# askerlee/AdaFace-dev

Hardware: AMD Instinct MI355X
Metric: denoise-steps/sec SD-1.5 U-Net 512px bs=4/GPU (higher is better)
Workload: dtype f16; 1 GPU; adaface_txt2img_ddim: SD-1.5 U-Net eps-prediction + CFG + DDIM update, 512x512 (latent 64x64), bs=4/GPU, U-Net batch 8 (cond+uncond), 77 tokens, DDIM-50 timesteps, random-init weights; parallelism=replicas x1, hipgraph=True, finite=True

## Files before the change

### adaface-dev_amd/_lib.py

```python
import ctypes as C
import os
import subprocess

_HERE = os.path.dirname(os.path.abspath(__file__))
CSRC = os.path.join(_HERE, "csrc")
LIB_PATH = os.environ.get("AF_LIB") or os.path.join(CSRC, "libadaface_hip.so")

AF_OK, AF_E_BADARG, AF_E_UNSUPPORTED, AF_E_HIP = 0, -1, -2, -3
AF_ACT_NONE, AF_ACT_SILU, AF_ACT_GEGLU, AF_ACT_QUICKGELU = 0, 1, 2, 3
AF_OUT_NORMAL, AF_OUT_SPLIT_T, AF_OUT_F32 = 0, 1, 2
AF_SPLITK_COUNTER_BYTES = 4096 * 4
AF_FAM_GEMM, AF_FAM_ATTN, AF_FAM_GNORM, AF_FAM_LNORM, AF_FAM_ELEM, AF_FAM_XATTN = 0, 1, 2, 3, 4, 5

EXPORTS = (
    "af_last_error", "af_version", "af_device_count", "af_prof_enable", "af_prof_reset", "af_prof_read",
    "af_gemm", "af_groupnorm_ws_floats", "af_groupnorm", "af_layernorm", "af_attention", "af_attention_scores",
    "af_timestep_embedding", "af_nchw_f32_to_nhwc_f16", "af_nhwc_f16_to_nchw_f32", "af_cfg_ddim_step", "af_q_sample",
    "af_silu_f16", "af_attention_lse", "af_groupnorm_stats", "af_attention_bwd_scratch_bytes", "af_attention_bwd",
    "af_groupnorm_bwd", "af_layernorm_bwd", "af_geglu_fwd", "af_geglu_bwd", "af_sumpool2x2", "af_add_f16",
    "af_transpose_tokens", "af_cadamw_step", "af_attention_ex", "af_colsum", "af_quickgelu_fwd", "af_quickgelu_bwd",
    "af_scale_f32", "af_affine_prelu", "af_maxpool2x2", "af_global_avgpool", "af_se_residual_prelu", "af_axpy_f16", "af_dora_combine", "af_mul_f16", "af_im2col3x3", "af_colsum_tall", "af_softmax_rows", "af_attention_strided", "af_clamp_f32", "af_mask_pairs", "af_prefetch", "af_prefetch_ex",
    "af_xattn_scores", "af_xattn_softmax_pv", "af_xattn_softmax_pv_bwd", "af_xattn_rowmix", "af_xattn_colmix_ws_bytes", "af_xattn_colmix",
    "af_layernorm_param_grads", "af_transpose_tokens_pair", "af_ff_fused", "af_ff_chain", "af_xattn_fused",
    "af_softmax_rows_bwd", "af_affine_prelu_bwd", "af_maxpool2x2_bwd", "af_se_gate_grad", "af_se_residual_prelu_bwd",
    "af_groupnorm_apply", "af_gemm_gn_stats_ok", "af_gemm_halo_variant", "af_gn_proj_fused",
    "af_xattn_chain",
    "af_image_u8_to_nhwc_f16", "af_vae_latents_q_sample", "af_cfg_dpmpp_step", "af_cfg_lcm_step",
    "af_cfg_ddim_inpaint_step", "af_cfg_dpmpp_inpaint_step", "af_cfg_lcm_inpaint_step", "af_vae_latents_z_q_sample",
    "af_vae_attention", "af_latent_resize_q_sample", "af_affine_prelu_ch", "af_face_align_crop",
    "af_stem_im2col7x7", "af_relu_maxpool3x3s2", "af_subsample2x", "af_upsample2x_add", "af_retina_decode", "af_retina_nms",
)


class GemmDesc(C.Structure):
    _fields_ = [
        ("a1", C.c_void_p), ("a2", C.c_void_p), ("wt", C.c_void_p), ("bias", C.c_void_p),
        ("rowbias", C.c_void_p), ("residual", C.c_void_p), ("out", C.c_void_p), ("out2", C.c_void_p),
        ("M", C.c_int32), ("N", C.c_int32), ("K", C.c_int32), ("kpad", C.c_int32), ("taps", C.c_int32),
        ("c1", C.c_int32), ("c2", C.c_int32), ("lda1", C.c_int32), ("lda2", C.c_int32),
        ("B", C.c_int32), ("H", C.c_int32), ("W", C.c_int32), ("Ho", C.c_int32), ("Wo", C.c_int32),
        ("stride", C.c_int32), ("upsample", C.c_int32), ("rows_per_batch", C.c_int32), ("ld_rowbias", C.c_int32),
        ("act", C.c_int32), ("out_mode", C.c_int32), ("ld_out", C.c_int32), ("split_col", C.c_int32),
        ("ld_out2", C.c_int32), ("tile", C.c_int32), ("splits", C.c_int32),
        ("workspace", C.c_void_p), ("workspace_bytes", C.c_int64), ("zeros", C.c_void_p),
        ("tap_shift", C.c_int32), ("splitk_fused", C.c_int32),
        ("ln_colsum", C.c_void_p), ("ln_eps", C.c_float),
        ("a3", C.c_void_p), ("a4", C.c_void_p), ("c3", C.c_int32), ("c4", C.c_int32), ("lda3", C.c_int32), ("lda4", C.c_int32),
        ("gn_partials", C.c_void_p), ("gn_cpg", C.c_int32),
# ... 46 lines not shown
        return _lib
    import torch
    if not os.path.exists(LIB_PATH):
        raise RuntimeError(
            f"{LIB_PATH} not found: the HIP extension is required (no CPU fallback). "
            "Run `python -c 'import __graft_entry__ as g; g.build()'` or `make -C adaface-dev_amd/csrc`."
        )
    L = C.CDLL(LIB_PATH)
    vp, i32, i64, f32 = C.c_void_p, C.c_int, C.c_int64, C.c_float
    L.af_last_error.restype = C.c_char_p
    L.af_last_error.argtypes = []
    L.af_version.argtypes = []
    L.af_device_count.argtypes = []
    L.af_prof_enable.argtypes = [i32]
    L.af_prof_reset.argtypes = []
    L.af_prof_read.argtypes = [i32, C.POINTER(C.c_int), C.POINTER(C.c_double)]
    L.af_gemm.argtypes = [C.POINTER(GemmDesc), vp]
    L.af_groupnorm_ws_floats.argtypes = [i32]
    L.af_groupnorm.argtypes = [vp, vp, i32, i32, vp, vp, vp, i32, i32, i32, f32, i32, vp, vp]
    L.af_groupnorm_apply.argtypes = [vp, i32, vp, vp, vp, vp, i32, i32, i32, f32, i32, vp, i32, vp]
    L.af_gemm_gn_stats_ok.argtypes = [i32, i32, i32, i32, i32, i32, i32, i32]
    L.af_gemm_halo_variant.argtypes = [C.POINTER(GemmDesc)]
    L.af_gn_proj_fused.argtypes = [vp, vp, i32, vp, vp, f32, vp, vp, i32, vp, i32, i32, i32, i32, vp, vp]
    L.af_layernorm.argtypes = [vp, vp, vp, vp, i32, i32, f32, vp]
    L.af_attention.argtypes = [vp, vp, vp, vp, vp, i32, i32, i32, i32, i32, i32, i32, i32, i32, i32, f32, vp]
    L.af_attention_scores.argtypes = [vp, vp, vp, vp, i32, i32, i32, i32, i32, f32, vp]
    L.af_timestep_embedding.argtypes = [vp, vp, i32, i32, f32, vp]
    L.af_nchw_f32_to_nhwc_f16.argtypes = [vp, vp, i32, i32, i32, i32, vp]
    L.af_nhwc_f16_to_nchw_f32.argtypes = [vp, vp, i32, i32, i32, i32, vp]
    L.af_cfg_ddim_step.argtypes = [vp, vp, vp, vp, i64, i32, f32, f32, f32, vp]
    L.af_cfg_dpmpp_step.argtypes = [vp, vp, vp, vp, vp, vp, i64, i32, f32, f32, f32, f32, f32, f32, vp]
    L.af_cfg_lcm_step.argtypes = [vp, vp, vp, vp, vp, i64, i32, f32, f32, f32, f32, f32, f32, f32, vp]
    L.af_q_sample.argtypes = [vp, vp, vp, vp, vp, i32, i64, vp]
    L.af_image_u8_to_nhwc_f16.argtypes = [vp, vp, i32, i32, i32, vp]
    L.af_vae_latents_q_sample.argtypes = [vp, vp, vp, vp, vp, f32, f32, f32, vp, i32, i32, i32, i32, vp]
    L.af_vae_latents_z_q_sample.argtypes = [vp, vp, vp, vp, vp, f32, f32, f32, vp, vp, i32, i32, i32, i32, vp]
    L.af_latent_resize_q_sample.argtypes = [vp, vp, vp, i32, i32, i32, i32, i32, i32, f32, f32, vp]
    blend = [vp, vp, vp, i32, i32, i64, f32, f32]
    L.af_cfg_ddim_inpaint_step.argtypes = L.af_cfg_ddim_step.argtypes[:-1] + blend + [vp]
    L.af_cfg_dpmpp_inpaint_step.argtypes = L.af_cfg_dpmpp_step.argtypes[:-1] + blend + [vp]
    L.af_cfg_lcm_inpaint_step.argtypes = L.af_cfg_lcm_step.argtypes[:-1] + blend + [vp]
    L.af_silu_f16.argtypes = [vp, vp, i64, vp]
    L.af_attention_lse.argtypes = [vp, vp, vp, vp, vp, i32, vp, i32, i32, i32, i32, i32, i32, i32, i32, i32, i32, f32, vp]
    L.af_attention_ex.argtypes = [vp, vp, vp, vp, vp, i32, vp, i32, i32, i32, i32, i32, i32, i32, i32, i32, i32, i32, f32, vp]
    L.af_attention_strided.argtypes = [vp, vp, vp, vp, vp, i32, vp, i32, i32, i32, i32, i32, i32, i32, i32, i32, i32, i32, i64, f32, vp]
    L.af_groupnorm_stats.argtypes = [vp, vp, i32, i32, vp, vp, vp, vp, i32, i32, i32, f32, i32, vp, vp]
# ... 68 lines not shown
```

### adaface-dev_amd/csrc/af_xattn_fused.hip

```cpp
#include <stdlib.h>

#include "af_common.h"

namespace {

__device__ __forceinline__ void glds16(const half_t* src, char* lds_dst) {
  __builtin_amdgcn_global_load_lds((const __attribute__((address_space(1))) void*)src,
                                   (__attribute__((address_space(3))) void*)lds_dst, 16, 0, 0);
}

constexpr int XA_C = 320, XA_H = 8, XA_D = 40, XA_BM = 128;
constexpr int XA_WQ = 5 * 48 * 128, XA_WO = XA_C * 128, XA_KB = 80 * 128, XA_VB = 2 * 48 * 128;
constexpr int XA_LDS = XA_WQ + 2 * (XA_WO + XA_KB + XA_VB) + 2 * XA_C * 4;

struct XaDev {
  const half_t* x;
  const half_t* wq;
  const float* bq;
  const float* cs;
  const half_t* k;
  const half_t* vt;
  const half_t* wo;
  const float* bo;
  const half_t* residual;
// ... 1039 lines not shown
#pragma unroll
      for (int tm = 0; tm < 4; ++tm) xf[tm] = *reinterpret_cast<const half8_t*>(Xs + frag_off(wm * 64 + tm * 16, kk));
#pragma unroll
      for (int tn = 0; tn < 5; ++tn)
#pragma unroll
        for (int tm = 0; tm < 4; ++tm) acc[tn][tm] = __builtin_amdgcn_mfma_f32_16x16x32_f16(wf[tn], xf[tm], acc[tn][tm], 0, 0, 0);
    }
  }
#pragma unroll
  for (int tm = 0; tm < 4; ++tm) {
    const int m = m0 + wm * 64 + tm * 16 + fr;
    if (m >= p.M) continue;
#pragma unroll
    for (int tn = 0; tn < 5; ++tn) {
      const int c = wn * 80 + tn * 16 + 4 * fq;
      floatx4 v = acc[tn][tm];
      if (p.bias) {
        const floatx4 b = *reinterpret_cast<const floatx4*>(p.bias + c);
#pragma unroll
        for (int e = 0; e < 4; ++e) v[e] += b[e];
      }
      const half4_t o = {(half_t)v[0], (half_t)v[1], (half_t)v[2], (half_t)v[3]};
      *reinterpret_cast<half4_t*>(p.out + (size_t)m * XA_C + c) = o;
    }
  }
}

}

extern "C" int af_xattn_fused(const void* x, const void* wq, const void* bq, const void* ln_colsum, float ln_eps, int kpad_q, const void* k, int ldk,
                              const void* vt, int64_t vt_batch_stride, int ldv, const void* wo, const void* bo, int kpad_o, const void* residual,
                              void* out, int B, int N, int L, int C, int heads, float scale, const void* zeros, void* stream) {
  AF_REQUIRE(x && wq && k && vt && wo && out && zeros, "af_xattn_fused: null pointer");
  AF_SUPPORTED((C == XA_C || C == X6_C) && heads == XA_H, "af_xattn_fused: built for C = 320 / 640, 8 heads (the 64 x 64 and 32 x 32 levels of SD-1.5)");
  AF_REQUIRE(B > 0 && N > 0 && N % (C == XA_C ? XA_BM : X6_BM) == 0, "af_xattn_fused: tokens per image must be a positive multiple of 128 (C = 320) / 64 (C = 640)");
  AF_SUPPORTED(L > 0 && L <= 80, "af_xattn_fused: at most 80 keys");
  AF_REQUIRE(kpad_q >= C && kpad_q % 64 == 0 && kpad_o >= C && kpad_o % 64 == 0, "af_xattn_fused: weight row strides must be 64-multiples covering C");
  AF_REQUIRE(ldk >= C && ldk % 8 == 0 && ldv >= L && ldv % 8 == 0 && vt_batch_stride % 8 == 0, "af_xattn_fused: K / V^T strides must keep 16-byte alignment");
  XaDev p{};
  p.x = (const half_t*)x;
  p.wq = (const half_t*)wq;
  p.bq = (const float*)bq;
  p.cs = (const float*)ln_colsum;
  p.ln_on = ln_colsum != nullptr;
  p.k = (const half_t*)k;
  p.vt = (const half_t*)vt;
// ... 92 lines not shown
  AF_REQUIRE(B > 0 && HW > 0 && HW % XA_BM == 0 && nblk == HW / XA_BM && nblk <= 128, "af_gn_proj_fused: HW must be a multiple of 128 (at most 128 blocks) and nblk = HW / 128");
  AF_REQUIRE(kpad >= C && kpad % 64 == 0, "af_gn_proj_fused: the weight row stride must be a 64-multiple covering C");
  AF_REQUIRE((((uintptr_t)x | (uintptr_t)out | (uintptr_t)gamma | (uintptr_t)beta | (uintptr_t)w) & 15) == 0, "af_gn_proj_fused: x / out / gamma / beta / w must be 16-byte aligned");
  GpDev p;
  p.x = (const half_t*)x;
  p.partials = (const float*)partials;
  p.gamma = (const float*)gamma;
  p.beta = (const float*)beta;
  p.w = (const half_t*)w;
  p.bias = (const float*)bias;
  p.out = (half_t*)out;
  p.zeros = (const half_t*)zeros;
  p.M = B * HW;
  p.HW = HW;
  p.nblk = nblk;
  p.kpad = kpad;
  p.eps = eps;
  static bool attr_set = false;
  if (!af_allow_dyn_lds(reinterpret_cast<const void*>(&af_gn_proj320_kernel), XT_LDS, attr_set, "af_gn_proj_fused")) return af_check_launch("af_gn_proj_fused");
  AfLaunchScope scope(AF_FAM_GEMM, stream);
  hipLaunchKernelGGL(af_gn_proj320_kernel, dim3(p.M / XA_BM), dim3(512), XT_LDS, (hipStream_t)stream, p);
  return af_check_launch("af_gn_proj_fused");
}
```

### adaface-dev_amd/ldm/modules/attention.py

```python
import math
import os as _os

import torch
import torch.nn as nn
import torch.nn.functional as F

from ... import ops
from ...ops import AF_ACT_GEGLU, F16
from .diffusionmodules.util import (Conv2d, GroupNorm32, LayerNorm, Linear, _PackCache, checkpoint, from_nhwc_f16,
                                    to_nhwc_f16, zero_module)


FOLD_LAYERNORM = _os.environ.get("AF_FOLD_LAYERNORM", "1") != "0"
FUSE_GN_PROJ = _os.environ.get("AF_FUSE_GN_PROJ", "1") != "0"
CHAIN_XATTN = _os.environ.get("AF_CHAIN_XATTN", "1") != "0"
XATTN_FUSE_MIN_TOKENS = int(_os.environ.get("AF_XATTN_FUSE_MIN_TOKENS", "8192"))
CHAIN_PROJ_OUT = _os.environ.get("AF_CHAIN_PROJ_OUT", "1") != "0"
FUSE_XATTN640 = _os.environ.get("AF_FUSE_XATTN640", "0") != "0"
XATTN640_FUSE_MIN_TOKENS = 4096
FUSE_XATTN = _os.environ.get("AF_FUSE_XATTN", "1") != "0"
FUSE_FF = _os.environ.get("AF_FUSE_FF", "1") != "0"


def exists(val):
    return val is not None


def default(val, d):
    if exists(val):
        return val
    return d() if callable(d) else d


def Normalize(in_channels):
    return GroupNorm32(num_groups=32, num_channels=in_channels, eps=1e-6, affine=True)


# ... 113 lines not shown
        ws = (self.to_k.weight, self.to_v.weight)
        return self._kv_cache.get(ws, lambda: ops.pack_matrix(torch.cat([w.detach() for w in ws], 0), None, ws[0].device))

    def _packed_qkv_ln(self, ln):
        ws = (self.to_q.weight, self.to_k.weight, self.to_v.weight)
        if not hasattr(self, "_qkv_cache_ln"):
            self._qkv_cache_ln = _PackCache()
        return self._qkv_cache_ln.get(ws + (ln.weight, ln.bias), lambda: ops.pack_matrix_ln(
            torch.cat([w.detach() for w in ws], 0), None, ln.weight, ln.bias, ln.eps, ws[0].device))

    def _packed_q_ln(self, ln):
        if not hasattr(self, "_q_cache_ln"):
            self._q_cache_ln = _PackCache()
        return self._q_cache_ln.get((self.to_q.weight, ln.weight, ln.bias), lambda: ops.pack_matrix_ln(
            self.to_q.weight, None, ln.weight, ln.bias, ln.eps, self.to_q.weight.device))

    def xattn_fusable(self, C, B, N, L, ln, chain=False) -> bool:
        if not (FUSE_XATTN and ln is not None and self.heads == 8 and not self.save_cross_attn_vars and L <= 80 and self.inner_dim == C):
            return False
        if C == 320:
            return N % 128 == 0 and B * N >= XATTN_FUSE_MIN_TOKENS
        return bool(FUSE_XATTN640 and not chain and C == 640 and N % 64 == 0 and B * N >= XATTN640_FUSE_MIN_TOKENS)

    def hip(self, x2d, B, N, context=None, keybias=None, residual=None, ln=None, defer_out=False, pre=None):
        Ci, h, d = self.inner_dim, self.heads, self.dim_head
        if context is None:
            if self.to_k.in_features != self.to_q.in_features:
                raise RuntimeError("CrossAttention: context is required (context_dim != query_dim)")
            L = N
            qk, vt = ops.gemm(x2d, self._packed_qkv() if ln is None else self._packed_qkv_ln(ln), rows_per_batch=N, split_col=2 * Ci)
            q, k, ldq, ldk = qk, qk[:, Ci:], 2 * Ci, 2 * Ci
        else:
            L = context.shape[1]
            ldk = Ci
            if self._kv_pre is not None:
                k, vt, ldk = self._kv_pre
            else:
                k, vt = ops.gemm(context.reshape(B * L, context.shape[-1]), self._packed_kv(), rows_per_batch=L, split_col=Ci)
            if pre is not None:
                ao, pw_o1, x0 = pre
                return ops.xattn_chain(ao, pw_o1, x0, self._packed_q_ln(ln), k, vt, self.to_out[0].packed(), B=B, N=N, L=L, heads=h, scale=self.scale, ldk=ldk)
            if keybias is None and self.xattn_fusable(x2d.shape[1], B, N, L, ln):
                return ops.xattn_fused(x2d, self._packed_q_ln(ln), k, vt, self.to_out[0].packed(), B=B, N=N, L=L, heads=h, scale=self.scale,
                                       ldk=ldk, residual=residual)
            q = self.to_q.hip(x2d) if ln is None else ops.gemm(x2d, self._packed_q_ln(ln))
            ldq = Ci
        o = ops.attention(q, k, vt, B=B, Nq=N, L=L, heads=h, d=d, ldq=ldq, ldk=ldk, keybias=keybias, scale=self.scale)
        if self.save_cross_attn_vars:
            out_plain = self.to_out[0].hip(o)
            qc = q if context is not None else qk[:, :Ci].contiguous()
            kc = k.contiguous() if context is not None else qk[:, Ci:].contiguous()
            score, prob = ops.attention_scores(qc, kc, B=B, Nq=N, L=L, heads=h, d=d, scale=self.scale)
            rs = math.sqrt(self.scale)
# ... 60 lines not shown
        return self.to_q.hip_dgrad(dq), dctx

    def forward(self, x, context=None, mask=None):
        B, N, _ = x.shape
        x2d = x.reshape(B * N, -1).to(F16).contiguous()
        ctx = None if context is None else context.to(F16).contiguous()
        L = N if ctx is None else ctx.shape[1]
        kb = None if mask is None else ops.make_keybias(mask.reshape(B, -1), L)
        y = self.hip(x2d, B, N, ctx, kb).reshape(B, N, -1)
        return y if x.dtype == F16 else y.to(x.dtype)


class BasicTransformerBlock(nn.Module):
    def __init__(self, dim, n_heads, d_head, dropout=0.0, context_dim=None, gated_ff=True, checkpoint=True):
        super().__init__()
        self.attn1 = CrossAttention(query_dim=dim, heads=n_heads, dim_head=d_head, dropout=dropout)
        self.ff = FeedForward(dim, dropout=dropout, glu=gated_ff)
        self.attn2 = CrossAttention(query_dim=dim, context_dim=context_dim, heads=n_heads, dim_head=d_head, dropout=dropout)
        self.norm1 = LayerNorm(dim)
        self.norm2 = LayerNorm(dim)
        self.norm3 = LayerNorm(dim)
        self.checkpoint = checkpoint

    def hip(self, x2d, B, N, context=None, keybias=None, post=None):
        if FOLD_LAYERNORM and x2d.shape[1] % 64 == 0:
            small = x2d.shape[0] < 1024
            if (CHAIN_XATTN and not small and context is not None and not self.attn1.save_cross_attn_vars 
                    and self.attn2.xattn_fusable(x2d.shape[1], B, N, context.shape[1], self.norm2, chain=True)):
                pre = self.attn1.hip(x2d, B, N, None, keybias, residual=x2d, ln=self.norm1, defer_out=True)
                x2 = self.attn2.hip(None, B, N, context, None, residual=None, ln=self.norm2, pre=pre)
                return self.ff.hip(x2, residual=x2, ln=self.norm3, post=post if self.post_done(x2d.shape[0], x2d.shape[1], post) else None)
            x1 = self.attn1.hip(self.norm1.hip(x2d) if small else x2d, B, N, None, keybias, residual=x2d, ln=None if small else self.norm1)
            x2 = self.attn2.hip(self.norm2.hip(x1) if small else x1, B, N, context, None, residual=x1, ln=None if small else self.norm2)
            return self.ff.hip(x2, residual=x2, ln=self.norm3, post=post if self.post_done(x2d.shape[0], x2d.shape[1], post) else None)
        x1 = self.attn1.hip(self.norm1.hip(x2d), B, N, None, keybias, residual=x2d)
        x2 = self.attn2.hip(self.norm2.hip(x1), B, N, context, None, residual=x1)
        return self.ff.hip(self.norm3.hip(x2), residual=x2)

    def post_done(self, M, C, post) -> bool:
        return bool(post is not None and CHAIN_PROJ_OUT and FOLD_LAYERNORM and C % 64 == 0 and self.ff.ff_fusable(M, C, self.norm3))

    def hip_train(self, x2d, B, N, context=None, keybias=None):
        if FOLD_LAYERNORM and x2d.shape[1] % 64 == 0 and x2d.shape[0] >= 1024:
            x1, s1 = self.attn1.hip_train(x2d, B, N, None, keybias, residual=x2d, ln=self.norm1)
            x2, s2 = self.attn2.hip_train(x1, B, N, context, None, residual=x1, ln=self.norm2)
            x3, hp = self.ff.hip_train(x2, residual=x2, ln=self.norm3)
            return x3, (x2d, x1, x2, s1, s2, hp)
        x1, s1 = self.attn1.hip_train(self.norm1.hip(x2d), B, N, None, keybias, residual=x2d)
        x2, s2 = self.attn2.hip_train(self.norm2.hip(x1), B, N, context, None, residual=x1)
        x3, hp = self.ff.hip_train(self.norm3.hip(x2), residual=x2)
        return x3, (x2d, x1, x2, s1, s2, hp)

    def hip_bwd(self, saved, dy, dctx=None):
        x, x1, x2, s1, s2, hp = saved
        dx2 = self.norm3.hip_bwd(x2, self.ff.hip_bwd(hp, dy), add=dy)
        dn2, dctx = self.attn2.hip_bwd(s2, dx2, dctx)
        dx1 = self.norm2.hip_bwd(x1, dn2, add=dx2)
# ... 17 lines not shown
        super().__init__()
        self.in_channels = in_channels
        inner_dim = n_heads * d_head
        self.norm = Normalize(in_channels)
        self.proj_in = Conv2d(in_channels, inner_dim, kernel_size=1, stride=1, padding=0)
        self.transformer_blocks = nn.ModuleList(
            [BasicTransformerBlock(inner_dim, n_heads, d_head, dropout=dropout, context_dim=context_dim) for _ in range(depth)]
        )
        self.proj_out = zero_module(Conv2d(inner_dim, in_channels, kernel_size=1, stride=1, padding=0))

    live_mask_rule = False

    def _keybias(self, mask, B, H, W):
        m2 = F.interpolate(mask.float(), size=(H, W), mode="nearest")
        kb = ops.make_keybias(m2.reshape(B, H * W), H * W)
        if self.live_mask_rule:
            any_empty = (m2.sum(dim=(2, 3)) == 0).any()
            kb = torch.where(any_empty, torch.zeros_like(kb), kb)
        return kb

    def hip(self, x, context=None, mask=None):
        B, H, W, Cn = x.shape
        N = H * W
        y = ops.gn_proj_fused(x, self.norm.weight, self.norm.bias, self.norm.eps, self.proj_in.packed(), self.norm.num_groups) if FUSE_GN_PROJ else None
        if y is None:
            y = self.norm.hip(x)
            y = self.proj_in.hip(y).reshape(B * N, -1)
        kb = None
        if mask is not None:
            kb = self._keybias(mask, B, H, W)
        cpg = Cn // 32 if Cn % 32 == 0 else 0
        last = len(self.transformer_blocks) - 1
        post = (self.proj_out.packed(), x.reshape(B * N, Cn), N, cpg)
        chained = False
        for i, block in enumerate(self.transformer_blocks):
            block.attn2.infeat_size = (H, W)
            if i == last and block.post_done(B * N, y.shape[1], post):
                y, chained = block.hip(y, B, N, context, kb, post=post), True
            else:
                y = block.hip(y, B, N, context, kb)
        out = y if chained else ops.gemm(y, self.proj_out.packed(), residual=x.reshape(B * N, Cn), rows_per_batch=N, gn_cpg=cpg)
        out4 = out.reshape(B, H, W, Cn)
        if hasattr(out, "_gn_partials"):
            out4._gn_partials = out._gn_partials
        return out4

    def hip_train(self, x, context=None, mask=None):
        B, H, W, Cn = x.shape
        N = H * W
        y, st = self.norm.hip_train(x)
        y = self.proj_in.hip(y).reshape(B * N, -1)
        kb = None
        if mask is not None:
            kb = self._keybias(mask, B, H, W)
        bs = []
        for block in self.transformer_blocks:
            block.attn2.infeat_size = (H, W)
            y, s = block.hip_train(y, B, N, context, kb)
            bs.append(s)
        out = ops.gemm(y, self.proj_out.packed(), residual=x.reshape(B * N, Cn))
        return out.reshape(B, H, W, Cn), (x, st, bs)

    def hip_bwd(self, saved, dy, dctx=None):
# ... 12 lines not shown
```

### adaface-dev_amd/ops.py

```python
import ctypes as C
from dataclasses import dataclass
from typing import Optional

import torch

from . import _lib
from ._lib import AF_ACT_GEGLU, AF_ACT_NONE, AF_ACT_QUICKGELU, AF_ACT_SILU, AF_OUT_F32, AF_OUT_NORMAL, AF_OUT_SPLIT_T, GemmDesc

F16 = torch.float16
NEG_MAX = -torch.finfo(torch.float32).max



def param_key(p):
    if p is None:
        return None
    gen = p.__dict__.get("_af_gen")
    return (p.data_ptr(), p._version, p.device, gen[0] if gen is not None else -1)


def _stream() -> int:
    return torch._C._cuda_getCurrentRawStream(torch._C._cuda_getDevice())


# ... 545 lines not shown
    if gn is not None and gn.B == B and gn.hw == hw and gn.C == c1 and gn.cpg * groups == c1 and x.is_contiguous():
        rc = _lib.lib().af_groupnorm_apply(_p(x), c1, _p(gamma), _p(beta), _p(y), _p(stats), B, hw, groups, float(eps), int(silu), _p(gn.ws), gn.nblk, _stream())
        _lib.check(rc, "af_groupnorm_apply")
        return y, stats
    ws = _gn_workspace(x.device, B)
    if stats is None:
        rc = _lib.lib().af_groupnorm(_p(x), _p(x2), c1, c2, _p(gamma), _p(beta), _p(y), B, hw, groups, float(eps), int(silu), _p(ws), _stream())
        _lib.check(rc, "af_groupnorm")
    else:
        rc = _lib.lib().af_groupnorm_stats(_p(x), _p(x2), c1, c2, _p(gamma), _p(beta), _p(y), _p(stats), B, hw, groups, float(eps), int(silu), _p(ws), _stream())
        _lib.check(rc, "af_groupnorm_stats")
    return y, stats


def groupnorm(x: torch.Tensor, gamma: torch.Tensor, beta: torch.Tensor, eps: float, silu: bool, *,
              x2: Optional[torch.Tensor] = None, groups: int = 32) -> torch.Tensor:
    return _groupnorm(x, gamma, beta, eps, silu, x2, groups, False)[0]


def groupnorm_train(x, gamma, beta, eps, silu, *, x2=None, groups=32):
    return _groupnorm(x, gamma, beta, eps, silu, x2, groups, True)


def gn_proj_fused(x: torch.Tensor, gamma: torch.Tensor, beta: torch.Tensor, eps: float, pw: PackedWeight, groups: int = 32) -> Optional[torch.Tensor]:
    gn = partials_of(x)
    B, c = x.shape[0], x.shape[-1]
    hw = x.numel() // (B * c)
    if (gn is None or c != 320 or groups != 32 or pw.N != 320 or pw.K != 320 or pw.ln_cs is not None or hw % 128 != 0 or gn.B != B or gn.hw != hw or gn.C != c
            or gn.cpg * groups != c or not x.is_contiguous()):
        return None
    _chk_f16(x, "gn_proj_fused.x")
    out = torch.empty((B * hw, pw.N), dtype=F16, device=x.device)
    _pf_note(pw.wt)
    rc = _lib.lib().af_gn_proj_fused(_p(x), _p(gn.ws), gn.nblk, _p(gamma), _p(beta), float(eps), _p(pw.wt), _p(pw.bias), pw.kpad, _p(out), B, hw, c, groups,
                                     _zero_page(x.device).data_ptr(), _stream())
    _lib.check(rc, "af_gn_proj_fused")
    return out


def layernorm(x: torch.Tensor, gamma: torch.Tensor, beta: torch.Tensor, eps: float = 1e-5) -> torch.Tensor:
    _chk_f16(x, "layernorm.x")
    Cn = x.shape[-1]
    y = torch.empty_like(x)
    _lib.check(_lib.lib().af_layernorm(_p(x), _p(gamma), _p(beta), _p(y), x.numel() // Cn, Cn, float(eps), _stream()),
               "af_layernorm")
    return y


def attention(q: torch.Tensor, k: torch.Tensor, vt: torch.Tensor, *, B: int, Nq: int, L: int, heads: int, d: int,
              ldq: int, ldk: int, keybias: Optional[torch.Tensor] = None, scale: Optional[float] = None,
              want_lse: bool = False, causal_m: int = 0):
    Cn = heads * d
    o = torch.empty((B * Nq, Cn), dtype=F16, device=q.device)
    scale = d ** -0.5 if scale is None else scale
    ldb = 0 if keybias is None else keybias.stride(0)
    lse = torch.empty((B, heads, round_up(Nq, 32)), dtype=torch.float32, device=q.device) if want_lse else None
    rc = _lib.lib().af_attention_strided(_p(q), _p(k), _p(vt), _p(o), _p(lse), 0 if lse is None else lse.stride(1), _p(keybias),
                                         int(causal_m), B, Nq, L, heads, d, ldq, ldk, Cn, vt.stride(1), ldb, vt.stride(0), float(scale),
                                         _stream())
    _lib.check(rc, "af_attention")
# ... 643 lines not shown
```

### include/adaface_hip.h

```cpp
#ifndef ADAFACE_HIP_H
#define ADAFACE_HIP_H

#include <stdint.h>

#ifdef __cplusplus
extern "C" {
#endif

#define AF_OK 0
#define AF_E_BADARG (-1)
#define AF_E_UNSUPPORTED (-2)
#define AF_E_HIP (-3)

const char* af_last_error(void);
int af_version(void);
int af_device_count(void);

#define AF_FAM_GEMM 0
#define AF_FAM_ATTN 1
#define AF_FAM_GNORM 2
#define AF_FAM_LNORM 3
#define AF_FAM_ELEM 4
#define AF_FAM_XATTN 5
#define AF_FAM_COUNT 6
// ... 53 lines not shown
#define AF_SPLITK_COUNTER_BYTES (AF_SPLITK_MAX_TILES * 4)

int af_gemm(const af_gemm_desc* d, void* stream);

int af_ff_fused(const void* x, const void* w1, const void* b1, const void* ln_colsum, float ln_eps, int kpad1, const void* w2, const void* b2,
                int kpad2, const void* residual, void* out, int M, int C, int inner, const void* zeros, void* stream);
int af_ff_chain(const void* x, const void* w1, const void* b1, const void* ln_colsum, float ln_eps, int kpad1, const void* w2, const void* b2, int kpad2,
                const void* residual, const void* wp, const void* bp, int kpad_p, const void* x_in, void* out, void* gn_partials, int gn_cpg,
                int rows_per_batch, int M, int C, int inner, const void* zeros, void* stream);

int af_xattn_fused(const void* x, const void* wq, const void* bq, const void* ln_colsum, float ln_eps, int kpad_q, const void* k, int ldk,
                   const void* vt, int64_t vt_batch_stride, int ldv, const void* wo, const void* bo, int kpad_o, const void* residual,
                   void* out, int B, int N, int L, int C, int heads, float scale, const void* zeros, void* stream);

int af_xattn_chain(const void* ao, const void* w1, const void* b1, int kpad_1, const void* x0, void* x1, const void* wq, const void* bq,
                   const void* ln_colsum, float ln_eps, int kpad_q, const void* k, int ldk, const void* vt, int64_t vt_batch_stride, int ldv,
                   const void* wo, const void* bo, int kpad_o, void* out, int B, int N, int L, int C, int heads, float scale, const void* zeros,
                   void* stream);


int af_gn_proj_fused(const void* x, const void* partials, int nblk, const void* gamma, const void* beta, float eps, const void* w, const void* bias,
                     int kpad, void* out, int B, int HW, int C, int groups, const void* zeros, void* stream);

int af_groupnorm_ws_floats(int B);
int af_groupnorm_apply(const void* x, int C, const void* gamma, const void* beta, void* y, void* stats, int B, int HW, int groups, float eps,
                       int silu, const void* partials, int nblk, void* stream);
int af_gemm_gn_stats_ok(int tile, int splits, int taps, int act, int out_mode, int N, int cpg, int rows_per_batch);
int af_gemm_halo_variant(const af_gemm_desc* d);
int af_groupnorm(const void* x1, const void* x2, int c1, int c2, const void* gamma, const void* beta,
                 void* y, int B, int HW, int groups, float eps, int silu, void* workspace, void* stream);

int af_groupnorm_stats(const void* x1, const void* x2, int c1, int c2, const void* gamma, const void* beta,
                       void* y, void* stats, int B, int HW, int groups, float eps, int silu, void* workspace,
                       void* stream);

int af_layernorm(const void* x, const void* gamma, const void* beta, void* y, int rows, int C, float eps,
                 void* stream);

int af_attention(const void* q, const void* k, const void* vt, void* o, const void* keybias, int B, int Nq,
                 int L, int heads, int d, int ldq, int ldk, int ldo, int ldv, int ldb, float scale, void* stream);
int af_attention_lse(const void* q, const void* k, const void* vt, void* o, void* lse2, int ld_lse, const void* keybias,
                     int B, int Nq, int L, int heads, int d, int ldq, int ldk, int ldo, int ldv, int ldb, float scale,
                     void* stream);

int af_attention_ex(const void* q, const void* k, const void* vt, void* o, void* lse2, int ld_lse, const void* keybias,
                    int causal_m, int B, int Nq, int L, int heads, int d, int ldq, int ldk, int ldo, int ldv, int ldb,
// ... 122 lines not shown
```

Before: 98.34 denoise-steps/s.

## Chain GroupNorm+proj_in with the first block's LayerNorm-folded QKV projection

Adds a fused HIP kernel for the 320-channel 64x64 level. It applies GroupNorm and proj_in, computes the per-row LayerNorm statistics from the proj_in tile kept in LDS, then runs the packed q|k|v projection with the folded LayerNorm and writes qk plus a transposed V. This avoids a separate QKV GEMM launch and re-reading the proj_in output from global memory for the first transformer block. In exchange the kernel computes LN statistics from the f16-rounded output, runs with 512 threads and one block per CU, and is gated by token count and shape checks.

```diff
diff --git a/adaface-dev_amd/_lib.py b/adaface-dev_amd/_lib.py
--- a/adaface-dev_amd/_lib.py
+++ b/adaface-dev_amd/_lib.py
@@ -23,7 +23,7 @@
     "af_xattn_scores", "af_xattn_softmax_pv", "af_xattn_softmax_pv_bwd", "af_xattn_rowmix", "af_xattn_colmix_ws_bytes", "af_xattn_colmix",
     "af_layernorm_param_grads", "af_transpose_tokens_pair", "af_ff_fused", "af_ff_chain", "af_xattn_fused",
     "af_softmax_rows_bwd", "af_affine_prelu_bwd", "af_maxpool2x2_bwd", "af_se_gate_grad", "af_se_residual_prelu_bwd",
-    "af_groupnorm_apply", "af_gemm_gn_stats_ok", "af_gemm_halo_variant", "af_gn_proj_fused",
+    "af_groupnorm_apply", "af_gemm_gn_stats_ok", "af_gemm_halo_variant", "af_gn_proj_fused", "af_gn_proj_qkv_chain",
     "af_xattn_chain",
     "af_image_u8_to_nhwc_f16", "af_vae_latents_q_sample", "af_cfg_dpmpp_step", "af_cfg_lcm_step",
     "af_cfg_ddim_inpaint_step", "af_cfg_dpmpp_inpaint_step", "af_cfg_lcm_inpaint_step", "af_vae_latents_z_q_sample",
@@ -116,6 +116,7 @@
     L.af_gemm_gn_stats_ok.argtypes = [i32, i32, i32, i32, i32, i32, i32, i32]
     L.af_gemm_halo_variant.argtypes = [C.POINTER(GemmDesc)]
     L.af_gn_proj_fused.argtypes = [vp, vp, i32, vp, vp, f32, vp, vp, i32, vp, i32, i32, i32, i32, vp, vp]
+    L.af_gn_proj_qkv_chain.argtypes = [vp, vp, i32, vp, vp, f32, vp, vp, i32, vp, vp, vp, vp, f32, i32, i32, vp, vp, i32, i32, i32, i32, i32, vp, vp]
     L.af_layernorm.argtypes = [vp, vp, vp, vp, i32, i32, f32, vp]
     L.af_attention.argtypes = [vp, vp, vp, vp, vp, i32, i32, i32, i32, i32, i32, i32, i32, i32, i32, f32, vp]
     L.af_attention_scores.argtypes = [vp, vp, vp, vp, i32, i32, i32, i32, i32, f32, vp]
diff --git a/adaface-dev_amd/csrc/af_xattn_fused.hip b/adaface-dev_amd/csrc/af_xattn_fused.hip
--- a/adaface-dev_amd/csrc/af_xattn_fused.hip
+++ b/adaface-dev_amd/csrc/af_xattn_fused.hip
@@ -1085,6 +1085,265 @@
       }
       const half4_t o = {(half_t)v[0], (half_t)v[1], (half_t)v[2], (half_t)v[3]};
       *reinterpret_cast<half4_t*>(p.out + (size_t)m * XA_C + c) = o;
+    }
+  }
+}
+
+struct GqDev {
+  GpDev g;
+  const half_t* wqkv;
+  const float* bqkv;
+  const float* cs;
+  half_t* qk;
+  half_t* vt;
+  int kpad_qkv, ldv;
+  float ln_eps;
+};
+
+__global__ __launch_bounds__(512, 1) void af_gn_proj_qkv320_kernel(const GqDev q) {
+  constexpr int NW = 8, G = 32, CPG = XA_C / G, NST = 20;
+  const GpDev& p = q.g;
+  extern __shared__ __attribute__((aligned(16))) char af_smem[];
+  char* R = af_smem;
+  char* RING = af_smem + XT_R;
+  const int tid = threadIdx.x, lane = tid & 63;
+  const int wave = __builtin_amdgcn_readfirstlane(tid >> 6);
+  const int prow = lane >> 3, slot = lane & 7;
+  const int fr = lane & 15, fq = lane >> 4;
+  const int m0 = blockIdx.x * XA_BM;
+  const int bimg = m0 / p.HW;
+  const floatx4 zf = {0.f, 0.f, 0.f, 0.f};
+  {
+    const int coop = gridDim.x < 32 ? (int)gridDim.x : 32;
+    af_prefetch_weight_tile(p.w, p.kpad, XA_C, 0, XA_C, 0, XA_C / 64, coop, blockIdx.x % coop, 1, NW, wave, lane, RING + XT_STAGE);
+    af_prefetch_weight_tile(q.wqkv, q.kpad_qkv, 3 * XA_C, 0, 3 * XA_C, 0, XA_C / 64, coop, blockIdx.x % coop, 1, NW, wave, lane, RING + XT_STAGE);
+  }
+  auto issue_w = [&](int ph, int st) {
+    char* dst = RING + ((ph + st) & 1) * XT_STAGE;
+    const half_t* src = ph == 0 ? p.w + st * 64 : q.wqkv + (size_t)(ph - 1) * XA_C * q.kpad_qkv + st * 64;
+    const int ld = ph == 0 ? p.kpad : q.kpad_qkv;
+#pragma unroll
+    for (int j = 0; j < 5; ++j) {
+      const int pc = wave + NW * j, row = pc * 8 + prow;
+      const int lc = slot ^ ((row >> 1) & 7);
+      glds16(src + (size_t)row * ld + lc * 8, dst + pc * 1024);
+    }
+  };
+  issue_w(0, 0);
+  const bool act = tid < 480;
+  const int ch = tid % 40, r0 = tid / 40;
+  half8_t xv[11];
+#pragma unroll
+  for (int k = 0; k < 11; ++k) {
+    const int r = r0 + 12 * k;
+    if (act && r < XA_BM && m0 + r < p.M) xv[k] = *reinterpret_cast<const half8_t*>(p.x + (size_t)(m0 + r) * XA_C + ch * 8);
+  }
+  floatx4 gm[2], bt[2];
+  if (act) {
+    gm[0] = *reinterpret_cast<const floatx4*>(p.gamma + ch * 8);
+    gm[1] = *reinterpret_cast<const floatx4*>(p.gamma + ch * 8 + 4);
+    bt[0] = *reinterpret_cast<const floatx4*>(p.beta + ch * 8);
+    bt[1] = *reinterpret_cast<const floatx4*>(p.beta + ch * 8 + 4);
+  }
+  float* fold = reinterpret_cast<float*>(R);
+  float* mr = fold + 16 * G * 3;
+  {
+    const int g = tid & 31, kl = tid >> 5;
+    GnAcc acc = {0.f, 0.f, 0.f};
+    for (int k = kl; k < p.nblk; k += 16) {
+      const float* w = p.partials + (((size_t)bimg * 128 + k) * G + g) * 2;
+      acc = gn_acc_merge(acc, GnAcc{128.f * CPG, w[0], w[1]});
+    }
+    fold[(kl * G + g) * 3] = acc.n;
+    fold[(kl * G + g) * 3 + 1] = acc.s;
+    fold[(kl * G + g) * 3 + 2] = acc.m2;
+  }
+  __syncthreads();
+  if (tid < G) {
+    GnAcc acc = {fold[tid * 3], fold[tid * 3 + 1], fold[tid * 3 + 2]};
+#pragma unroll
+    for (int k = 1; k < 16; ++k) acc = gn_acc_merge(acc, GnAcc{fold[(k * G + tid) * 3], fold[(k * G + tid) * 3 + 1], fold[(k * G + tid) * 3 + 2]});
+    const float inv_n = 1.0f / ((float)p.HW * (float)CPG);
+    const float mean = acc.s * inv_n;
+    const float var = fmaxf(acc.m2 * inv_n, 0.f);
+    mr[tid * 2] = mean;
+    mr[tid * 2 + 1] = rsqrtf(var + p.eps);
+  }
+  __syncthreads();
+  float sc[8], sh[8];
+  if (act) {
+#pragma unroll
+    for (int e = 0; e < 8; ++e) {
+      const int g = (ch * 8 + e) / CPG;
+      const float k = mr[g * 2 + 1] * gm[e >> 2][e & 3];
+      sc[e] = k;
+      sh[e] = bt[e >> 2][e & 3] - mr[g * 2] * k;
+    }
+  }
+  __syncthreads();
+  if (act) {
+#pragma unroll
+    for (int k = 0; k < 11; ++k) {
+      const int r = r0 + 12 * k;
+      if (r < XA_BM) {
+        half8_t o = {0, 0, 0, 0, 0, 0, 0, 0};
+        if (m0 + r < p.M) {
+#pragma unroll
+          for (int e = 0; e < 8; ++e) o[e] = (half_t)((float)xv[k][e] * sc[e] + sh[e]);
+        }
+        *reinterpret_cast<half8_t*>(R + (ch >> 3) * (XA_BM * 128) + r * 128 + (((ch & 7) ^ ((r >> 1) & 7)) * 16)) = o;
+      }
+    }
+  }
+  auto lds_barrier = [&]() {
+    asm volatile("s_waitcnt lgkmcnt(0)" ::: "memory");
+    __builtin_amdgcn_s_barrier();
+    asm volatile("" ::: "memory");
+  };
+  auto frag_off = [&](int row0, int kk) { return (row0 + fr) * 128 + (((kk * 4 + fq) ^ (((row0 + fr) >> 1) & 7)) * 16); };
+  const int wm = wave & 1, wn = wave >> 1;
+  float mean[4] = {0.f, 0.f, 0.f, 0.f}, rstd[4] = {1.f, 1.f, 1.f, 1.f};
+#pragma nounroll
+  for (int ph = 0; ph < 4; ++ph) {
+    floatx4 acc[5][4];
+#pragma unroll
+    for (int tn = 0; tn < 5; ++tn)
+#pragma unroll
+      for (int tm = 0; tm < 4; ++tm) acc[tn][tm] = zf;
+#pragma nounroll
+    for (int st = 0; st < 5; ++st) {
+      const int g = ph * 5 + st;
+      asm volatile("s_waitcnt vmcnt(0) lgkmcnt(0)" ::: "memory");
+      __builtin_amdgcn_s_barrier();
+      if (g + 1 < NST) issue_w(st == 4 ? ph + 1 : ph, st == 4 ? 0 : st + 1);
+      const char* Ws = RING + (g & 1) * XT_STAGE;
+      const char* Xs = R + st * (XA_BM * 128);
+#pragma unroll
+      for (int kk = 0; kk < 2; ++kk) {
+        half8_t wf[5], xf[4];
+#pragma unroll
+        for (int tn = 0; tn < 5; ++tn) wf[tn] = *reinterpret_cast<const half8_t*>(Ws + frag_off(wn * 80 + tn * 16, kk));
+#pragma unroll
+        for (int tm = 0; tm < 4; ++tm) xf[tm] = *reinterpret_cast<const half8_t*>(Xs + frag_off(wm * 64 + tm * 16, kk));
+#pragma unroll
+        for (int tn = 0; tn < 5; ++tn)
+#pragma unroll
+          for (int tm = 0; tm < 4; ++tm) acc[tn][tm] = __builtin_amdgcn_mfma_f32_16x16x32_f16(wf[tn], xf[tm], acc[tn][tm], 0, 0, 0);
+      }
+    }
+    floatx4 csv[5], bv[5];
+    {
+      const float* bsrc = ph == 0 ? p.bias : q.bqkv;
+      const int n0 = (ph > 0 ? (ph - 1) * XA_C : 0) + wn * 80 + 4 * fq;
+#pragma unroll
+      for (int tn = 0; tn < 5; ++tn) {
+        bv[tn] = bsrc ? *reinterpret_cast<const floatx4*>(bsrc + n0 + tn * 16) : zf;
+        csv[tn] = ph == 0 ? zf : *reinterpret_cast<const floatx4*>(q.cs + n0 + tn * 16);
+      }
+    }
+    if (ph == 0) {
+      lds_barrier();
+#pragma unroll
+      for (int tm = 0; tm < 4; ++tm) {
+        const int row = wm * 64 + tm * 16 + fr, m = m0 + row;
+#pragma unroll
+        for (int tn = 0; tn < 5; ++tn) {
+          const int c = wn * 80 + tn * 16 + 4 * fq;
+          floatx4 v = acc[tn][tm];
+#pragma unroll
+          for (int e = 0; e < 4; ++e) v[e] += bv[tn][e];
+          const half4_t o = {(half_t)v[0], (half_t)v[1], (half_t)v[2], (half_t)v[3]};
+          if (m < p.M) *reinterpret_cast<half4_t*>(p.out + (size_t)m * XA_C + c) = o;
+          *reinterpret_cast<half4_t*>(R + (c >> 6) * (XA_BM * 128) + row * 128 + ((((c & 63) >> 3) ^ ((row >> 1) & 7)) * 16) + ((c >> 2) & 1) * 8) = o;
+        }
+      }
+      lds_barrier();
+      float* lnst = reinterpret_cast<float*>(RING);
+      {
+        const half2_t one2 = {(half_t)1.0f, (half_t)1.0f};
+        float s = 0.f, qq = 0.f;
+#pragma unroll
+        for (int c = 0; c < 5; ++c) {
+          const half8_t f0 = *reinterpret_cast<const half8_t*>(R + c * (XA_BM * 128) + frag_off(wave * 16, 0));
+          const half8_t f1 = *reinterpret_cast<const half8_t*>(R + c * (XA_BM * 128) + frag_off(wave * 16, 1));
+#pragma unroll
+          for (int e = 0; e < 8; e += 2) {
+            const half2_t a = {f0[e], f0[e + 1]}, b = {f1[e], f1[e + 1]};
+            s = __builtin_amdgcn_fdot2(a, one2, s, false);
+            qq = __builtin_amdgcn_fdot2(a, a, qq, false);
+            s = __builtin_amdgcn_fdot2(b, one2, s, false);
+            qq = __builtin_amdgcn_fdot2(b, b, qq, false);
+          }
+        }
+        s += __shfl_xor(s, 16, 64);
+        qq += __shfl_xor(qq, 16, 64);
+        s += __shfl_xor(s, 32, 64);
+        qq += __shfl_xor(qq, 32, 64);
+        if (fq == 0) {
+          const float mu = s * (1.0f / XA_C), var = fmaxf(qq * (1.0f / XA_C) - mu * mu, 0.f);
+          lnst[2 * (wave * 16 + fr)] = mu;
+          lnst[2 * (wave * 16 + fr) + 1] = rsqrtf(var + q.ln_eps);
+        }
+      }
+      lds_barrier();
+#pragma unroll
+      for (int tm = 0; tm < 4; ++tm) {
+        const int row = wm * 64 + tm * 16 + fr;
+        mean[tm] = lnst[2 * row];
+        rstd[tm] = lnst[2 * row + 1];
+      }
+    } else if (ph < 3) {
+#pragma unroll
+      for (int tm = 0; tm < 4; ++tm) {
+        const int m = m0 + wm * 64 + tm * 16 + fr;
+        if (m >= p.M) continue;
+#pragma unroll
+        for (int tn = 0; tn < 5; ++tn) {
+          const int c = (ph - 1) * XA_C + wn * 80 + tn * 16 + 4 * fq;
+          floatx4 v;
+#pragma unroll
+          for (int e = 0; e < 4; ++e) {
+            const float a = rstd[tm] * (acc[tn][tm][e] - mean[tm] * csv[tn][e]);
+            v[e] = a + bv[tn][e];
+          }
+          const half4_t o = {(half_t)v[0], (half_t)v[1], (half_t)v[2], (half_t)v[3]};
+          *reinterpret_cast<half4_t*>(q.qk + (size_t)m * (2 * XA_C) + c) = o;
+        }
+      }
+    } else {
+      constexpr int TT = XA_BM + 8;
+      static_assert(XA_C * TT * 2 <= XT_LDS, "the transposed V tile is staged over R + ring");
+      lds_barrier();
+      half_t* T = reinterpret_cast<half_t*>(af_smem);
+#pragma unroll
+      for (int tm = 0; tm < 4; ++tm) {
+        const int row = wm * 64 + tm * 16 + fr;
+        const bool mok = m0 + row < p.M;
+#pragma unroll
+        for (int tn = 0; tn < 5; ++tn) {
+          const int col = wn * 80 + tn * 16 + 4 * fq;
+#pragma unroll
+          for (int e = 0; e < 4; ++e) {
+            const float a = rstd[tm] * (acc[tn][tm][e] - mean[tm] * csv[tn][e]);
+            T[(col + e) * TT + row] = mok ? (half_t)(a + bv[tn][e]) : (half_t)0.f;
+          }
+        }
+      }
+      __syncthreads();
+      const int tok0 = m0 - bimg * p.HW;
+      half_t* o2 = q.vt + (size_t)bimg * XA_C * q.ldv + tok0;
+      constexpr int CPC = XA_BM / 8;
+      for (int c = tid; c < XA_C * CPC; c += 64 * NW) {
+        const int col = c / CPC, cc = c - col * CPC;
+        if (m0 + cc * 8 < p.M) *reinterpret_cast<half8_t*>(o2 + (size_t)col * q.ldv + cc * 8) = *reinterpret_cast<const half8_t*>(T + col * TT + cc * 8);
+      }
+      if (tok0 + XA_BM == p.HW && q.ldv > p.HW) {
+        const int padn = q.ldv - p.HW;
+        for (int c = tid; c < XA_C * padn; c += 64 * NW) {
+          const int col = c / padn, t = c - col * padn;
+          o2[(size_t)col * q.ldv + XA_BM + t] = (half_t)0.f;
+        }
+      }
     }
   }
 }
@@ -1223,3 +1482,48 @@
   hipLaunchKernelGGL(af_gn_proj320_kernel, dim3(p.M / XA_BM), dim3(512), XT_LDS, (hipStream_t)stream, p);
   return af_check_launch("af_gn_proj_fused");
 }
+
+extern "C" int af_gn_proj_qkv_chain(const void* x, const void* partials, int nblk, const void* gamma, const void* beta, float eps, const void* w, const void* bias,
+                                    int kpad, void* out, const void* wqkv, const void* bqkv, const void* ln_colsum, float ln_eps, int kpad_qkv, int n_qkv, void* qk,
+                                    void* vt, int ldv, int B, int HW, int C, int groups, const void* zeros, void* stream) {
+  AF_REQUIRE(x && partials && gamma && beta && w && out && wqkv && qk && vt && zeros, "af_gn_proj_qkv_chain: null pointer");
+  AF_SUPPORTED(C == XA_C && groups == 32, "af_gn_proj_qkv_chain: built for C = 320 in 32 groups (the 64 x 64 level of SD-1.5)");
+  AF_SUPPORTED(B > 0 && HW > 0 && HW % XA_BM == 0 && HW / XA_BM <= 128 && (long)B * HW < (1l << 31) / (3 * XA_C),
+               "af_gn_proj_qkv_chain: HW must be a multiple of 128 (at most 128 blocks per batch item)");
+  AF_REQUIRE(nblk == HW / XA_BM, "af_gn_proj_qkv_chain: nblk = HW / 128");
+  AF_SUPPORTED(n_qkv == 3 * XA_C && ln_colsum != nullptr, "af_gn_proj_qkv_chain: the q | k | v weight must be 960 x 320 packed with a folded LayerNorm");
+  AF_SUPPORTED(kpad >= C && kpad % 64 == 0 && kpad_qkv >= C && kpad_qkv % 64 == 0, "af_gn_proj_qkv_chain: weight row strides must be 64-multiples covering C");
+  AF_REQUIRE(ldv >= HW && ldv % 8 == 0, "af_gn_proj_qkv_chain: ldv must be a multiple of 8 covering HW");
+  AF_REQUIRE((((uintptr_t)x | (uintptr_t)out | (uintptr_t)gamma | (uintptr_t)beta | (uintptr_t)w | (uintptr_t)bias | (uintptr_t)wqkv | (uintptr_t)bqkv |
+               (uintptr_t)ln_colsum | (uintptr_t)qk | (uintptr_t)vt | (uintptr_t)partials | (uintptr_t)zeros) & 15) == 0,
+             "af_gn_proj_qkv_chain: every pointer must be 16-byte aligned");
+  AF_REQUIRE(out != x && qk != x && vt != x && qk != out && vt != out && vt != qk, "af_gn_proj_qkv_chain: out / qk / vt must be buffers of their own");
+  GqDev q;
+  GpDev& p = q.g;
+  p.x = (const half_t*)x;
+  p.partials = (const float*)partials;
+  p.gamma = (const float*)gamma;
+  p.beta = (const float*)beta;
+  p.w = (const half_t*)w;
+  p.bias = (const float*)bias;
+  p.out = (half_t*)out;
+  p.zeros = (const half_t*)zeros;
+  p.M = B * HW;
+  p.HW = HW;
+  p.nblk = nblk;
+  p.kpad = kpad;
+  p.eps = eps;
+  q.wqkv = (const half_t*)wqkv;
+  q.bqkv = (const float*)bqkv;
+  q.cs = (const float*)ln_colsum;
+  q.qk = (half_t*)qk;
+  q.vt = (half_t*)vt;
+  q.kpad_qkv = kpad_qkv;
+  q.ldv = ldv;
+  q.ln_eps = ln_eps;
+  static bool attr_set = false;
+  if (!af_allow_dyn_lds(reinterpret_cast<const void*>(&af_gn_proj_qkv320_kernel), XT_LDS, attr_set, "af_gn_proj_qkv_chain")) return af_check_launch("af_gn_proj_qkv_chain");
+  AfLaunchScope scope(AF_FAM_GEMM, stream);
+  hipLaunchKernelGGL(af_gn_proj_qkv320_kernel, dim3(p.M / XA_BM), dim3(512), XT_LDS, (hipStream_t)stream, q);
+  return af_check_launch("af_gn_proj_qkv_chain");
+}
diff --git a/adaface-dev_amd/ldm/modules/attention.py b/adaface-dev_amd/ldm/modules/attention.py
--- a/adaface-dev_amd/ldm/modules/attention.py
+++ b/adaface-dev_amd/ldm/modules/attention.py
@@ -13,6 +13,8 @@
 
 FOLD_LAYERNORM = _os.environ.get("AF_FOLD_LAYERNORM", "1") != "0"
 FUSE_GN_PROJ = _os.environ.get("AF_FUSE_GN_PROJ", "1") != "0"
+CHAIN_GN_QKV = _os.environ.get("AF_CHAIN_GN_QKV", "1") != "0"
+CHAIN_GN_QKV_MIN_TOKENS = int(_os.environ.get("AF_CHAIN_GN_QKV_MIN_TOKENS", "24576"))
 CHAIN_XATTN = _os.environ.get("AF_CHAIN_XATTN", "1") != "0"
 XATTN_FUSE_MIN_TOKENS = int(_os.environ.get("AF_XATTN_FUSE_MIN_TOKENS", "8192"))
 CHAIN_PROJ_OUT = _os.environ.get("AF_CHAIN_PROJ_OUT", "1") != "0"
@@ -172,13 +174,16 @@
             return N % 128 == 0 and B * N >= XATTN_FUSE_MIN_TOKENS
         return bool(FUSE_XATTN640 and not chain and C == 640 and N % 64 == 0 and B * N >= XATTN640_FUSE_MIN_TOKENS)
 
-    def hip(self, x2d, B, N, context=None, keybias=None, residual=None, ln=None, defer_out=False, pre=None):
+    def hip(self, x2d, B, N, context=None, keybias=None, residual=None, ln=None, defer_out=False, pre=None, qkv=None):
         Ci, h, d = self.inner_dim, self.heads, self.dim_head
         if context is None:
             if self.to_k.in_features != self.to_q.in_features:
                 raise RuntimeError("CrossAttention: context is required (context_dim != query_dim)")
             L = N
-            qk, vt = ops.gemm(x2d, self._packed_qkv() if ln is None else self._packed_qkv_ln(ln), rows_per_batch=N, split_col=2 * Ci)
+            if qkv is not None:
+                qk, vt = qkv
+            else:
+                qk, vt = ops.gemm(x2d, self._packed_qkv() if ln is None else self._packed_qkv_ln(ln), rows_per_batch=N, split_col=2 * Ci)
             q, k, ldq, ldk = qk, qk[:, Ci:], 2 * Ci, 2 * Ci
         else:
             L = context.shape[1]
@@ -285,17 +290,18 @@
         self.norm3 = LayerNorm(dim)
         self.checkpoint = checkpoint
 
-    def hip(self, x2d, B, N, context=None, keybias=None, post=None):
+    def hip(self, x2d, B, N, context=None, keybias=None, post=None, qkv=None):
         if FOLD_LAYERNORM and x2d.shape[1] % 64 == 0:
             small = x2d.shape[0] < 1024
             if (CHAIN_XATTN and not small and context is not None and not self.attn1.save_cross_attn_vars 
                     and self.attn2.xattn_fusable(x2d.shape[1], B, N, context.shape[1], self.norm2, chain=True)):
-                pre = self.attn1.hip(x2d, B, N, None, keybias, residual=x2d, ln=self.norm1, defer_out=True)
+                pre = self.attn1.hip(x2d, B, N, None, keybias, residual=x2d, ln=self.norm1, defer_out=True, qkv=qkv)
                 x2 = self.attn2.hip(None, B, N, context, None, residual=None, ln=self.norm2, pre=pre)
                 return self.ff.hip(x2, residual=x2, ln=self.norm3, post=post if self.post_done(x2d.shape[0], x2d.shape[1], post) else None)
-            x1 = self.attn1.hip(self.norm1.hip(x2d) if small else x2d, B, N, None, keybias, residual=x2d, ln=None if small else self.norm1)
+            x1 = self.attn1.hip(self.norm1.hip(x2d) if small and qkv is None else x2d, B, N, None, keybias, residual=x2d, ln=None if small else self.norm1, qkv=qkv)
             x2 = self.attn2.hip(self.norm2.hip(x1) if small else x1, B, N, context, None, residual=x1, ln=None if small else self.norm2)
             return self.ff.hip(x2, residual=x2, ln=self.norm3, post=post if self.post_done(x2d.shape[0], x2d.shape[1], post) else None)
+        assert qkv is None, "BasicTransformerBlock.hip: ready q | k | v projections come with the folded LayerNorm only"
         x1 = self.attn1.hip(self.norm1.hip(x2d), B, N, None, keybias, residual=x2d)
         x2 = self.attn2.hip(self.norm2.hip(x1), B, N, context, None, residual=x1)
         return self.ff.hip(self.norm3.hip(x2), residual=x2)
@@ -359,7 +365,16 @@
     def hip(self, x, context=None, mask=None):
         B, H, W, Cn = x.shape
         N = H * W
-        y = ops.gn_proj_fused(x, self.norm.weight, self.norm.bias, self.norm.eps, self.proj_in.packed(), self.norm.num_groups) if FUSE_GN_PROJ else None
+        y, qkv = None, None
+        b0 = self.transformer_blocks[0]
+        if (FUSE_GN_PROJ and CHAIN_GN_QKV and FOLD_LAYERNORM and Cn == 320 and N % 128 == 0 and B * N >= CHAIN_GN_QKV_MIN_TOKENS and ops.partials_of(x) is not None
+                and not b0.attn1.save_cross_attn_vars and b0.attn1.inner_dim == 320
+                and b0.attn1.to_q.in_features == 320 and b0.attn1.to_k.in_features == 320):
+            r = ops.gn_proj_qkv_chain(x, self.norm.weight, self.norm.bias, self.norm.eps, self.proj_in.packed(), b0.attn1._packed_qkv_ln(b0.norm1), self.norm.num_groups)
+            if r is not None:
+                y, qkv = r[0], (r[1], r[2])
+        if y is None and FUSE_GN_PROJ:
+            y = ops.gn_proj_fused(x, self.norm.weight, self.norm.bias, self.norm.eps, self.proj_in.packed(), self.norm.num_groups)
         if y is None:
             y = self.norm.hip(x)
             y = self.proj_in.hip(y).reshape(B * N, -1)
@@ -373,9 +388,9 @@
         for i, block in enumerate(self.transformer_blocks):
             block.attn2.infeat_size = (H, W)
             if i == last and block.post_done(B * N, y.shape[1], post):
-                y, chained = block.hip(y, B, N, context, kb, post=post), True
+                y, chained = block.hip(y, B, N, context, kb, post=post, qkv=qkv if i == 0 else None), True
             else:
-                y = block.hip(y, B, N, context, kb)
+                y = block.hip(y, B, N, context, kb, qkv=qkv if i == 0 else None)
         out = y if chained else ops.gemm(y, self.proj_out.packed(), residual=x.reshape(B * N, Cn), rows_per_batch=N, gn_cpg=cpg)
         out4 = out.reshape(B, H, W, Cn)
         if hasattr(out, "_gn_partials"):
diff --git a/adaface-dev_amd/ops.py b/adaface-dev_amd/ops.py
--- a/adaface-dev_amd/ops.py
+++ b/adaface-dev_amd/ops.py
@@ -591,20 +591,36 @@
     return _groupnorm(x, gamma, beta, eps, silu, x2, groups, True)
 
 
-def gn_proj_fused(x: torch.Tensor, gamma: torch.Tensor, beta: torch.Tensor, eps: float, pw: PackedWeight, groups: int = 32) -> Optional[torch.Tensor]:
+def gn_proj_fused(x: torch.Tensor, gamma: torch.Tensor, beta: torch.Tensor, eps: float, pw: PackedWeight, groups: int = 32, chain: Optional[PackedWeight] = None):
     gn = partials_of(x)
     B, c = x.shape[0], x.shape[-1]
     hw = x.numel() // (B * c)
     if (gn is None or c != 320 or groups != 32 or pw.N != 320 or pw.K != 320 or pw.ln_cs is not None or hw % 128 != 0 or gn.B != B or gn.hw != hw or gn.C != c
             or gn.cpg * groups != c or not x.is_contiguous()):
         return None
+    if chain is not None and (chain.N != 960 or chain.K != 320 or chain.ln_cs is None or chain.kpad % 64 != 0 or hw // 128 > 128):
+        return None
     _chk_f16(x, "gn_proj_fused.x")
     out = torch.empty((B * hw, pw.N), dtype=F16, device=x.device)
-    _pf_note(pw.wt)
-    rc = _lib.lib().af_gn_proj_fused(_p(x), _p(gn.ws), gn.nblk, _p(gamma), _p(beta), float(eps), _p(pw.wt), _p(pw.bias), pw.kpad, _p(out), B, hw, c, groups,
-                                     _zero_page(x.device).data_ptr(), _stream())
-    _lib.check(rc, "af_gn_proj_fused")
-    return out
+    if chain is None:
+        _pf_note(pw.wt)
+        rc = _lib.lib().af_gn_proj_fused(_p(x), _p(gn.ws), gn.nblk, _p(gamma), _p(beta), float(eps), _p(pw.wt), _p(pw.bias), pw.kpad, _p(out), B, hw, c, groups,
+                                         _zero_page(x.device).data_ptr(), _stream())
+        _lib.check(rc, "af_gn_proj_fused")
+        return out
+    qk = torch.empty((B * hw, 640), dtype=F16, device=x.device)
+    ldv = round_up(hw, 8)
+    vt = torch.empty((B, 320, ldv), dtype=F16, device=x.device)
+    _pf_note(pw.wt, chain.wt)
+    rc = _lib.lib().af_gn_proj_qkv_chain(_p(x), _p(gn.ws), gn.nblk, _p(gamma), _p(beta), float(eps), _p(pw.wt), _p(pw.bias), pw.kpad, _p(out), _p(chain.wt),
+                                         _p(chain.bias), _p(chain.ln_cs), float(chain.ln_eps), chain.kpad, chain.N, _p(qk), _p(vt), ldv, B, hw, c, groups,
+                                         _zero_page(x.device).data_ptr(), _stream())
+    _lib.check(rc, "af_gn_proj_qkv_chain")
+    return out, qk, vt
+
+
+def gn_proj_qkv_chain(x: torch.Tensor, gamma: torch.Tensor, beta: torch.Tensor, eps: float, pw_in: PackedWeight, pw_qkv_ln: PackedWeight, groups: int = 32):
+    return gn_proj_fused(x, gamma, beta, eps, pw_in, groups, chain=pw_qkv_ln)
 
 
 def layernorm(x: torch.Tensor, gamma: torch.Tensor, beta: torch.Tensor, eps: float = 1e-5) -> torch.Tensor:
diff --git a/include/adaface_hip.h b/include/adaface_hip.h
--- a/include/adaface_hip.h
+++ b/include/adaface_hip.h
@@ -99,6 +99,10 @@
 int af_gn_proj_fused(const void* x, const void* partials, int nblk, const void* gamma, const void* beta, float eps, const void* w, const void* bias,
                      int kpad, void* out, int B, int HW, int C, int groups, const void* zeros, void* stream);
 
+int af_gn_proj_qkv_chain(const void* x, const void* partials, int nblk, const void* gamma, const void* beta, float eps, const void* w, const void* bias,
+                         int kpad, void* out, const void* wqkv, const void* bqkv, const void* ln_colsum, float ln_eps, int kpad_qkv, int n_qkv, void* qk,
+                         void* vt, int ldv, int B, int HW, int C, int groups, const void* zeros, void* stream);
+
 int af_groupnorm_ws_floats(int B);
 int af_groupnorm_apply(const void* x, int C, const void* gamma, const void* beta, void* y, void* stats, int B, int HW, int groups, float eps,
                        int silu, const void* partials, int nblk, void* stream);
```

Result: no change. 99.09 denoise-steps/s, median of 6 (+0.8%).
